# JasonHopeSpace/panda

Measured on AMD Instinct MI355X. Metric: MSM points/s (BN254, 2^24), higher is better.
Workload: dtype u32; 1 GPU; BN254 MSM 2^24 points per GPU, Jacobian output, bases and scalars resident in HBM; curve=bn254, log_points_per_gpu=24, exchange=none

## Files before the change

panda_amd/csrc/curve29.h:

```cpp
#pragma once
#include "fe29.h"

namespace panda29 {

template <class F>
struct Xyzz {
    Fe<F> X, Y, ZZ, ZZZ;
};

template <class F>
struct Bounds {
    static constexpr int M = SubMargin<F>::value;
    static constexpr int XB = 8 + M;
    static constexpr int YB = SubGrowth<F, 2>::value;
    static constexpr int PB = 2 + SubGrowth<F, XB>::value;
    static constexpr int RB = 2 + SubGrowth<F, YB>::value;
    static constexpr int VB = 2 + SubGrowth<F, XB>::value;
    static constexpr long long LIM = F::HEADROOM * 9 / 10;
    static_assert((long long)PB * PB < LIM, "P^2 exceeds the lazy-reduction headroom");
    static constexpr int NB = SubGrowth<F, 2>::value;
    static_assert((long long)RB * VB + (long long)YB * NB < LIM, "R*(Q-X3) - Y1*PPP exceeds the lazy-reduction headroom");
    static_assert(6LL * VB + 2LL * NB < LIM, "3x^2*(S-X3) - W*Y exceeds the lazy-reduction headroom");
    static_assert((long long)(2 * YB) * (2 * YB) < LIM, "(2Y)^2 exceeds the lazy-reduction headroom");
    static_assert(2 + SubGrowth<F, 6>::value <= XB, "X3 bound");
// ... 110 lines not shown
    fe_mul(U2, bx, acc.ZZ);
    fe_sub<F, B::XB>(P, U2, acc.X);
    fe_mul(S2, by, acc.ZZZ);
    fe_sub<F, B::YB>(R, S2, acc.Y);
    fe_sqr(PP, P);
    if (fe_is_zero_2p(PP))
        return fe_is_zero_mod_p(R) ? 1 : 2;
    fe_mul(PPP, P, PP);
    fe_mul(Q, acc.X, PP);
    fe_mul(acc.ZZ, acc.ZZ, PP);
    fe_mul(acc.ZZZ, acc.ZZZ, PPP);
    xyzz_finish(X3, Y3, R, Q, PPP, acc.Y);
    acc.X = X3;
    acc.Y = Y3;
    return 0;
}

template <class F>
struct SignedBounds {
    static constexpr double H = (double)F::HEADROOM;
    static constexpr double XS = 4.4, XN = 3.2, YS = 2.0, ZS = 2.0;
    static constexpr double XM = XS > XN ? XS : XN;
    static constexpr double PS = XM + ZS / H + 1, RS = YS + ZS / H + 1;
    static constexpr double PPS = PS * PS / H + 1, P3S = PS * PPS / H + 1, QS = XM * PPS / H + 1;
    static constexpr double RRS = RS * RS / H + 1, VS = QS + XM;
    static_assert(PPS < 2, "PP must stay below 2p for fe_is_zero_2p");
    static_assert(2 * QS + P3S < XN && RRS + 2 * QS + P3S < XS, "X3 leaves the accumulator's bound");
    static_assert((RS * VS + YS * P3S) / H + 1 < YS, "Y3 leaves the accumulator's bound");
    static_assert(ZS * PPS / H + 1 < ZS && ZS * P3S / H + 1 < ZS, "ZZ, ZZZ leave the accumulator's bound");
    static constexpr int KX = 4, KY = 1, KZZZ = 1;
    static_assert(XN < KX - 0.5 && XS + KX <= Bounds<F>::XB, "stored X after the conversion");
    static_assert((RS * VS + YS * P3S) / H < KY - 0.5 && YS + KY <= Bounds<F>::YB, "stored Y after the conversion");
    static_assert(ZS * P3S / H < KZZZ - 0.5 && ZS + KZZZ <= 3, "stored ZZZ after the conversion");
};

template <class F>
PANDA_HD void signed_after_doubling(Xyzz<F> &acc)
{
    fe_reduce_small_2p(acc.X);
}

template <class F>
PANDA_HD int xyzz_madd_core_s(Xyzz<F> &acc, const Fe<F> &bx, const Fe<F> &by)
{
    typedef SignedBounds<F> B;
    (void)sizeof(B);
    Fe<F> U2, S2, P, R, PP, PPP, Q, X3, Y3, t, rr, v, nppp;
    fe_mul(U2, bx, acc.ZZ);
    fe_sub_s(P, U2, acc.X);
    fe_mul_s(S2, by, acc.ZZZ);
    fe_sub_s(R, S2, acc.Y);
    fe_sqr_s(PP, P);
    if (fe_is_zero_2p(PP))
        return fe_is_zero_mod_p_s(R) ? 1 : 2;
    fe_mul_s(PPP, P, PP);
    fe_mul_s(Q, acc.X, PP);
    fe_mul(acc.ZZ, acc.ZZ, PP);
    fe_mul_s(acc.ZZZ, acc.ZZZ, PPP);
    fe_sqr_s(rr, R);
#if defined(__HIP_DEVICE_COMPILE__)
#pragma unroll
    for (int i = 0; i < F::N; i++) asm volatile("" : "+v"(Q.l[i]), "+v"(PPP.l[i]) : "v"(rr.l[F::N - 1]));
#endif
    fe_add_nr(t, Q, Q);
    fe_add_nr(t, t, PPP);
    fe_sub_s_wide(X3, rr, t);
    fe_norm_s(X3, X3);
    fe_sub_s(v, Q, X3);
    fe_neg_s(nppp, PPP);
    fe_mul_add_s(Y3, R, v, acc.Y, nppp);
    acc.X = X3;
    acc.Y = Y3;
    return 0;
}

template <class F>
PANDA_HD void xyzz_madd(Xyzz<F> &acc, const Fe<F> &bx, const Fe<F> &by, bool base_identity)
{
    if (base_identity) return;
    if (xyzz_is_identity(acc)) {
        xyzz_from_affine(acc, bx, by);
        return;
    }
    const int rare = xyzz_madd_core(acc, bx, by);
    if (rare == 1)
        xyzz_dbl_affine(acc, bx, by);
    else if (rare == 2)
        xyzz_set_identity(acc);
}

template <class F>
struct OutlineRareDoubling {
    static constexpr bool value = IsExt2<F>::value && F::N > 18;
};
template <class F>
#if defined(__HIPCC__)
__host__ __device__
#endif
__attribute__((noinline)) void xyzz_dbl_noinline(Xyzz<F> &r, const Xyzz<F> &p)
{
    xyzz_dbl(r, p);
}

template <class F>
PANDA_HD void xyzz_add(Xyzz<F> &acc, const Xyzz<F> &q)
{
// ... 118 lines not shown
```

panda_amd/csrc/fe29.h:

```cpp
#pragma once
#include <stdint.h>

#include "fe29_params.h"

#if defined(__HIPCC__)
#define PANDA_HD __host__ __device__ inline __attribute__((always_inline))
#else
#define PANDA_HD inline __attribute__((always_inline))
#endif

#if defined(FE29_CHECK)
#include <assert.h>
#define FE29_SHADOW_DECL unsigned __int128 shadow = 0;
#define FE29_SHADOW_MAC(x, y) shadow += (unsigned __int128)(x) * (y);
#define FE29_SHADOW_SHIFT()                                      \
    assert(shadow < ((unsigned __int128)1 << 64) && "fe29 column accumulator overflow"); \
    shadow >>= 29;
#else
#define FE29_SHADOW_DECL
#define FE29_SHADOW_MAC(x, y)
#define FE29_SHADOW_SHIFT()
#endif

#if defined(__HIP_DEVICE_COMPILE__) && !defined(FE29_NO_ASM)
// ... 204 lines not shown
template <class F, int K>
__device__ inline __attribute__((always_inline)) void fe29_mul_add_col_s(uint64_t &acc, const uint32_t *a, const uint32_t *b, const uint32_t *c, const uint32_t *d, uint32_t *m,
                                                                         uint32_t *out)
{
    constexpr int N = F::N;
    if constexpr (K == 0) {
        MacChain<1>::vvi0(acc, a, b);
        MacChain<1>::vvi(acc, c, d);
    } else if constexpr (K < N) {
        MacChain<K + 1>::vvi(acc, a, b + K);
        MacChain<K + 1>::vvi(acc, c, d + K);
    } else {
        MacChain<2 * N - 1 - K>::vvi(acc, a + (K - N + 1), b + (N - 1));
        MacChain<2 * N - 1 - K>::vvi(acc, c + (K - N + 1), d + (N - 1));
    }
    fe29_reduce_col<F, K, true>(acc, m, out);
}
template <class F, int... K>
__device__ inline __attribute__((always_inline)) void fe29_mul_cols_s(uint64_t &acc, const uint32_t *a, const uint32_t *b, uint32_t *m, uint32_t *out, std::integer_sequence<int, K...>)
{
    (fe29_mul_col_s<F, K>(acc, a, b, m, out), ...);
}
template <class F, int... K>
__device__ inline __attribute__((always_inline)) void fe29_sqr_cols_s(uint64_t &acc, const uint32_t *a, const uint32_t *a2, uint32_t *m, uint32_t *out, std::integer_sequence<int, K...>)
{
    (fe29_sqr_col_s<F, K>(acc, a, a2, m, out), ...);
}
template <class F, int... K>
__device__ inline __attribute__((always_inline)) void fe29_mul_add_cols_s(uint64_t &acc, const uint32_t *a, const uint32_t *b, const uint32_t *c, const uint32_t *d,
                                                                          uint32_t *m, uint32_t *out, std::integer_sequence<int, K...>)
{
    (fe29_mul_add_col_s<F, K>(acc, a, b, c, d, m, out), ...);
}
#endif

template <class F>
PANDA_HD void fe_mul(Fe<F> &r, const Fe<F> &a, const Fe<F> &b)
{
    constexpr int N = F::N;
    u32 m[N];
    u32 out[N];
    u64 acc = 0;
#if defined(FE29_DEVICE_CHAINS)
    fe29_mul_cols<F>(acc, a.l, b.l, m, out, std::make_integer_sequence<int, 2 * N - 1>());
    out[N - 1] = (u32)acc;
#pragma unroll
    for (int i = 0; i < N; i++) r.l[i] = out[i];
    return;
#endif
    FE29_SHADOW_DECL
#pragma unroll
    for (int k = 0; k < N; k++) {
#pragma unroll
        for (int i = 0; i <= k; i++) {
            FE29_MAC(acc, a.l[i], b.l[k - i]);
            FE29_SHADOW_MAC(a.l[i], b.l[k - i])
        }
#pragma unroll
        for (int i = 0; i < k; i++) {
            FE29_MAC_CONST(acc, m[i], F::P[k - i]);
            FE29_SHADOW_MAC(m[i], F::P[k - i])
        }
        m[k] = ((u32)acc * F::INV) & LIMB_MASK;
        FE29_MAC_CONST(acc, m[k], F::P[0]);
        FE29_SHADOW_MAC(m[k], F::P[0])
        acc >>= LIMB_BITS;
// ... 267 lines not shown
template <class F, int KB>
struct SubGrowth {
    static constexpr int value = F::KEFF[KB + SubMargin<F>::value];
};

template <class F, int KB>
PANDA_HD void fe_neg(Fe<F> &r, const Fe<F> &a)
{
    if constexpr (IsExt2<F>::value) {
        fe_neg<typename F::Base, KB>(ext_c0(r), ext_c0(a));
        fe_neg<typename F::Base, KB>(ext_c1(r), ext_c1(a));
        return;
    } else {
    constexpr int K = KB + SubMargin<F>::value;
    Fe<F> t;
#pragma unroll
    for (int i = 0; i < F::N; i++) {
#if defined(FE29_CHECK)
        assert(F::KP[K][i] >= a.l[i] && "fe_neg limb range");
#endif
        t.l[i] = F::KP[K][i] - a.l[i];
    }
    fe_norm(r, t);
    }
}

template <class F>
struct SignedLimbsOk {
    static constexpr bool value = !IsExt2<F>::value && F::N <= 9;
};
template <class F>
PANDA_HD constexpr bool fe_signed_columns_fit()
{
    return 2ull * F::N * ((u64)SLIMB_MAX * SLIMB_MAX) + (u64)F::N * (1ull << 58) + (1ull << 35) < (1ull << 63);
}

template <class F>
PANDA_HD void fe_mul_s(Fe<F> &r, const Fe<F> &a, const Fe<F> &b)
{
    constexpr int N = F::N;
    static_assert(SignedLimbsOk<F>::value && fe_signed_columns_fit<F>(), "signed column accumulator too narrow");
    u32 m[N];
    u32 out[N];
    u64 acc = 0;
#if defined(FE29_DEVICE_CHAINS)
    fe29_mul_cols_s<F>(acc, a.l, b.l, m, out, std::make_integer_sequence<int, 2 * N - 1>());
    out[N - 1] = (u32)acc;
#pragma unroll
    for (int i = 0; i < N; i++) r.l[i] = out[i];
    return;
#endif
    FE29_SHADOW_DECL_S
#pragma unroll
    for (int i = 0; i < N; i++) {
        FE29_CHECK_SLIMB(a.l[i]);
        FE29_CHECK_SLIMB(b.l[i]);
    }
#pragma unroll
    for (int k = 0; k < N; k++) {
#pragma unroll
        for (int i = 0; i <= k; i++) {
            FE29_MAC_S(acc, a.l[i], b.l[k - i]);
            FE29_SHADOW_MAC_S(a.l[i], b.l[k - i])
        }
#pragma unroll
        for (int i = 0; i < k; i++) {
            FE29_MAC_CONST(acc, m[i], F::P[k - i]);
// ... 129 lines not shown
        }
        m[k] = ((u32)acc * F::INV) & LIMB_MASK;
        FE29_MAC_CONST(acc, m[k], F::P[0]);
        FE29_SHADOW_MAC_S(m[k], F::P[0])
        FE29_SHADOW_SHIFT_S()
        acc = (u64)((int64_t)acc >> LIMB_BITS);
    }
#pragma unroll
    for (int k = N; k < 2 * N - 1; k++) {
#pragma unroll
        for (int i = k - N + 1; 2 * i < k; i++) {
            FE29_MAC_S(acc, a2[i], a.l[k - i]);
            FE29_SHADOW_MAC_S(a2[i], a.l[k - i])
        }
        if ((k & 1) == 0) {
            FE29_MAC_S(acc, a.l[k / 2], a.l[k / 2]);
            FE29_SHADOW_MAC_S(a.l[k / 2], a.l[k / 2])
        }
#pragma unroll
        for (int i = k - N + 1; i < N; i++) {
            FE29_MAC_CONST(acc, m[i], F::P[k - i]);
            FE29_SHADOW_MAC_S(m[i], F::P[k - i])
        }
        out[k - N] = (u32)acc & LIMB_MASK;
        FE29_SHADOW_SHIFT_S()
        acc = (u64)((int64_t)acc >> LIMB_BITS);
    }
    out[N - 1] = (u32)acc;
#pragma unroll
    for (int i = 0; i < N; i++) r.l[i] = out[i];
}

template <class F>
PANDA_HD void fe_sub_s(Fe<F> &r, const Fe<F> &a, const Fe<F> &b)
{
    static_assert(SignedLimbsOk<F>::value, "signed limbs: 9-limb prime fields only");
#pragma unroll
    for (int i = 0; i < F::N; i++) {
        r.l[i] = a.l[i] - b.l[i];
        FE29_CHECK_SLIMB(r.l[i]);
    }
}

template <class F>
PANDA_HD void fe_sub_s_wide(Fe<F> &r, const Fe<F> &a, const Fe<F> &b)
{
    static_assert(SignedLimbsOk<F>::value, "signed limbs: 9-limb prime fields only");
#pragma unroll
    for (int i = 0; i < F::N; i++) r.l[i] = a.l[i] - b.l[i];
}

template <class F>
PANDA_HD void fe_neg_s(Fe<F> &r, const Fe<F> &a)
{
    static_assert(SignedLimbsOk<F>::value, "signed limbs: 9-limb prime fields only");
#pragma unroll
    for (int i = 0; i < F::N; i++) r.l[i] = 0u - a.l[i];
}

template <class F>
PANDA_HD void fe_norm_s(Fe<F> &r, const Fe<F> &t)
{
    constexpr int N = F::N;
    static_assert(SignedLimbsOk<F>::value, "signed limbs: 9-limb prime fields only");
    u32 c[N];
#pragma unroll
    for (int i = 0; i < N - 1; i++) {
        c[i] = (u32)((int32_t)t.l[i] >> LIMB_BITS);
#if defined(FE29_CHECK)
        assert((int32_t)c[i] >= -3 && (int32_t)c[i] <= 1 && "fe_norm_s carry range");
#endif
    }
    u32 o[N];
    o[0] = t.l[0] & LIMB_MASK;
#pragma unroll
    for (int i = 1; i < N - 1; i++) o[i] = (t.l[i] & LIMB_MASK) + c[i - 1];
    o[N - 1] = t.l[N - 1] + c[N - 2];
#pragma unroll
    for (int i = 0; i < N; i++) r.l[i] = o[i];
}

template <class F>
PANDA_HD bool fe_is_zero_mod_p_s(const Fe<F> &a)
{
    static_assert(F::HEADROOM >= 160, "the bound above is BN254-like: R / p >= 160");
    Fe<F> one, t;
    fe_one(one);
    fe_mul_s(t, a, one);
    return fe_is_zero_2p(t);
}

template <class F, int K>
PANDA_HD void fe_from_signed(Fe<F> &r, const Fe<F> &a)
{
    static_assert(SignedLimbsOk<F>::value && K >= 1 && K <= 200, "signed limbs: 9-limb prime fields only");
    Fe<F> t;
#pragma unroll
    for (int i = 0; i < F::N; i++) {
#if defined(FE29_CHECK)
        assert((int64_t)(int32_t)a.l[i] + (int64_t)F::KP[K][i] >= 0 && (int64_t)(int32_t)a.l[i] + (int64_t)F::KP[K][i] < (1ll << 32) && "fe_from_signed limb range");
#endif
        t.l[i] = a.l[i] + F::KP[K][i];
    }
    fe_norm(r, t);
}

template <class F>
PANDA_HD void fe_unpack(Fe<F> &r, const u32 *w)
{
    constexpr int N = F::N, L = F::L;
#pragma unroll
    for (int k = 0; k < N; k++) {
        const int bit = 29 * k, wi = bit >> 5, sh = bit & 31;
        u32 v = 0;
        if (wi < L) {
            v = w[wi] >> sh;
            if (sh > 3 && wi + 1 < L) v |= w[wi + 1] << (32 - sh);
        }
        r.l[k] = (k < N - 1) ? (v & LIMB_MASK) : v;
    }
}

template <class F>
PANDA_HD void fe_pack(u32 *w, const Fe<F> &a)
{
    constexpr int N = F::N, L = F::L;
#pragma unroll
    for (int i = 0; i < L; i++) {
        const int bit = 32 * i, j = bit / 29, s = bit - 29 * j;
        u32 v = a.l[j] >> s;
        if (j + 1 < N) v |= a.l[j + 1] << (29 - s);
        if (29 - s + 29 < 32 && j + 2 < N) v |= a.l[j + 2] << (58 - s);
        w[i] = v;
    }
}
// ... 400 lines not shown
```

panda_amd/csrc/fe29_chain.h:

```cpp
#pragma once
#include <stdint.h>

namespace panda29 {

template <int CNT>
struct MacChain;

template <>
struct MacChain<1> {
    static __device__ inline __attribute__((always_inline)) void vv(uint64_t &acc, const uint32_t *x, const uint32_t *y)
    {
        asm("v_mad_u64_u32 %0, vcc, %1, %2, %0" : "+v"(acc) : "v"(x[0]), "v"(y[0]) : "vcc");
    }
    static __device__ inline __attribute__((always_inline)) void vs(uint64_t &acc, const uint32_t *x, const uint32_t *y)
    {
        asm("v_mad_u64_u32 %0, vcc, %1, %2, %0" : "+v"(acc) : "v"(x[0]), "s"(y[0]) : "vcc");
    }
    static __device__ inline __attribute__((always_inline)) void vv0(uint64_t &acc, const uint32_t *x, const uint32_t *y)
    {
        asm("v_mad_u64_u32 %0, vcc, %1, %2, 0" : "=&v"(acc) : "v"(x[0]), "v"(y[0]) : "vcc");
    }
    static __device__ inline __attribute__((always_inline)) void vs0(uint64_t &acc, const uint32_t *x, const uint32_t *y)
    {
        asm("v_mad_u64_u32 %0, vcc, %1, %2, 0" : "=&v"(acc) : "v"(x[0]), "s"(y[0]) : "vcc");
// ... 338 lines not shown
        asm("v_mad_u64_u32 %0, vcc, %1, %2, %0\n\tv_mad_u64_u32 %0, vcc, %3, %4, %0\n\tv_mad_u64_u32 %0, vcc, %5, %6, %0\n\tv_mad_u64_u32 %0, vcc, %7, %8, %0\n\tv_mad_u64_u32 %0, vcc, %9, %10, %0\n\tv_mad_u64_u32 %0, vcc, %11, %12, %0\n\tv_mad_u64_u32 %0, vcc, %13, %14, %0\n\tv_mad_u64_u32 %0, vcc, %15, %16, %0\n\tv_mad_u64_u32 %0, vcc, %17, %18, %0\n\tv_mad_u64_u32 %0, vcc, %19, %20, %0\n\tv_mad_u64_u32 %0, vcc, %21, %22, %0\n\tv_mad_u64_u32 %0, vcc, %23, %24, %0\n\tv_mad_u64_u32 %0, vcc, %25, %26, %0\n\tv_mad_u64_u32 %0, vcc, %27, %28, %0" : "+v"(acc) : "v"(x[0]), "v"(y[0]), "v"(x[1]), "v"(y[-1]), "v"(x[2]), "v"(y[-2]), "v"(x[3]), "v"(y[-3]), "v"(x[4]), "v"(y[-4]), "v"(x[5]), "v"(y[-5]), "v"(x[6]), "v"(y[-6]), "v"(x[7]), "v"(y[-7]), "v"(x[8]), "v"(y[-8]), "v"(x[9]), "v"(y[-9]), "v"(x[10]), "v"(y[-10]), "v"(x[11]), "v"(y[-11]), "v"(x[12]), "v"(y[-12]), "v"(x[13]), "v"(y[-13]) : "vcc");
    }
    static __device__ inline __attribute__((always_inline)) void vs(uint64_t &acc, const uint32_t *x, const uint32_t *y)
    {
        asm("v_mad_u64_u32 %0, vcc, %1, %2, %0\n\tv_mad_u64_u32 %0, vcc, %3, %4, %0\n\tv_mad_u64_u32 %0, vcc, %5, %6, %0\n\tv_mad_u64_u32 %0, vcc, %7, %8, %0\n\tv_mad_u64_u32 %0, vcc, %9, %10, %0\n\tv_mad_u64_u32 %0, vcc, %11, %12, %0\n\tv_mad_u64_u32 %0, vcc, %13, %14, %0\n\tv_mad_u64_u32 %0, vcc, %15, %16, %0\n\tv_mad_u64_u32 %0, vcc, %17, %18, %0\n\tv_mad_u64_u32 %0, vcc, %19, %20, %0\n\tv_mad_u64_u32 %0, vcc, %21, %22, %0\n\tv_mad_u64_u32 %0, vcc, %23, %24, %0\n\tv_mad_u64_u32 %0, vcc, %25, %26, %0\n\tv_mad_u64_u32 %0, vcc, %27, %28, %0" : "+v"(acc) : "v"(x[0]), "s"(y[0]), "v"(x[1]), "s"(y[-1]), "v"(x[2]), "s"(y[-2]), "v"(x[3]), "s"(y[-3]), "v"(x[4]), "s"(y[-4]), "v"(x[5]), "s"(y[-5]), "v"(x[6]), "s"(y[-6]), "v"(x[7]), "s"(y[-7]), "v"(x[8]), "s"(y[-8]), "v"(x[9]), "s"(y[-9]), "v"(x[10]), "s"(y[-10]), "v"(x[11]), "s"(y[-11]), "v"(x[12]), "s"(y[-12]), "v"(x[13]), "s"(y[-13]) : "vcc");
    }
    static __device__ inline __attribute__((always_inline)) void vv0(uint64_t &acc, const uint32_t *x, const uint32_t *y)
    {
        asm("v_mad_u64_u32 %0, vcc, %1, %2, 0\n\tv_mad_u64_u32 %0, vcc, %3, %4, %0\n\tv_mad_u64_u32 %0, vcc, %5, %6, %0\n\tv_mad_u64_u32 %0, vcc, %7, %8, %0\n\tv_mad_u64_u32 %0, vcc, %9, %10, %0\n\tv_mad_u64_u32 %0, vcc, %11, %12, %0\n\tv_mad_u64_u32 %0, vcc, %13, %14, %0\n\tv_mad_u64_u32 %0, vcc, %15, %16, %0\n\tv_mad_u64_u32 %0, vcc, %17, %18, %0\n\tv_mad_u64_u32 %0, vcc, %19, %20, %0\n\tv_mad_u64_u32 %0, vcc, %21, %22, %0\n\tv_mad_u64_u32 %0, vcc, %23, %24, %0\n\tv_mad_u64_u32 %0, vcc, %25, %26, %0\n\tv_mad_u64_u32 %0, vcc, %27, %28, %0" : "=&v"(acc) : "v"(x[0]), "v"(y[0]), "v"(x[1]), "v"(y[-1]), "v"(x[2]), "v"(y[-2]), "v"(x[3]), "v"(y[-3]), "v"(x[4]), "v"(y[-4]), "v"(x[5]), "v"(y[-5]), "v"(x[6]), "v"(y[-6]), "v"(x[7]), "v"(y[-7]), "v"(x[8]), "v"(y[-8]), "v"(x[9]), "v"(y[-9]), "v"(x[10]), "v"(y[-10]), "v"(x[11]), "v"(y[-11]), "v"(x[12]), "v"(y[-12]), "v"(x[13]), "v"(y[-13]) : "vcc");
    }
    static __device__ inline __attribute__((always_inline)) void vs0(uint64_t &acc, const uint32_t *x, const uint32_t *y)
    {
        asm("v_mad_u64_u32 %0, vcc, %1, %2, 0\n\tv_mad_u64_u32 %0, vcc, %3, %4, %0\n\tv_mad_u64_u32 %0, vcc, %5, %6, %0\n\tv_mad_u64_u32 %0, vcc, %7, %8, %0\n\tv_mad_u64_u32 %0, vcc, %9, %10, %0\n\tv_mad_u64_u32 %0, vcc, %11, %12, %0\n\tv_mad_u64_u32 %0, vcc, %13, %14, %0\n\tv_mad_u64_u32 %0, vcc, %15, %16, %0\n\tv_mad_u64_u32 %0, vcc, %17, %18, %0\n\tv_mad_u64_u32 %0, vcc, %19, %20, %0\n\tv_mad_u64_u32 %0, vcc, %21, %22, %0\n\tv_mad_u64_u32 %0, vcc, %23, %24, %0\n\tv_mad_u64_u32 %0, vcc, %25, %26, %0\n\tv_mad_u64_u32 %0, vcc, %27, %28, %0" : "=&v"(acc) : "v"(x[0]), "s"(y[0]), "v"(x[1]), "s"(y[-1]), "v"(x[2]), "s"(y[-2]), "v"(x[3]), "s"(y[-3]), "v"(x[4]), "s"(y[-4]), "v"(x[5]), "s"(y[-5]), "v"(x[6]), "s"(y[-6]), "v"(x[7]), "s"(y[-7]), "v"(x[8]), "s"(y[-8]), "v"(x[9]), "s"(y[-9]), "v"(x[10]), "s"(y[-10]), "v"(x[11]), "s"(y[-11]), "v"(x[12]), "s"(y[-12]), "v"(x[13]), "s"(y[-13]) : "vcc");
    }
    static __device__ inline __attribute__((always_inline)) void vvi(uint64_t &acc, const uint32_t *x, const uint32_t *y)
    {
        asm("v_mad_i64_i32 %0, vcc, %1, %2, %0\n\tv_mad_i64_i32 %0, vcc, %3, %4, %0\n\tv_mad_i64_i32 %0, vcc, %5, %6, %0\n\tv_mad_i64_i32 %0, vcc, %7, %8, %0\n\tv_mad_i64_i32 %0, vcc, %9, %10, %0\n\tv_mad_i64_i32 %0, vcc, %11, %12, %0\n\tv_mad_i64_i32 %0, vcc, %13, %14, %0\n\tv_mad_i64_i32 %0, vcc, %15, %16, %0\n\tv_mad_i64_i32 %0, vcc, %17, %18, %0\n\tv_mad_i64_i32 %0, vcc, %19, %20, %0\n\tv_mad_i64_i32 %0, vcc, %21, %22, %0\n\tv_mad_i64_i32 %0, vcc, %23, %24, %0\n\tv_mad_i64_i32 %0, vcc, %25, %26, %0\n\tv_mad_i64_i32 %0, vcc, %27, %28, %0" : "+v"(acc) : "v"(x[0]), "v"(y[0]), "v"(x[1]), "v"(y[-1]), "v"(x[2]), "v"(y[-2]), "v"(x[3]), "v"(y[-3]), "v"(x[4]), "v"(y[-4]), "v"(x[5]), "v"(y[-5]), "v"(x[6]), "v"(y[-6]), "v"(x[7]), "v"(y[-7]), "v"(x[8]), "v"(y[-8]), "v"(x[9]), "v"(y[-9]), "v"(x[10]), "v"(y[-10]), "v"(x[11]), "v"(y[-11]), "v"(x[12]), "v"(y[-12]), "v"(x[13]), "v"(y[-13]) : "vcc");
    }
    static __device__ inline __attribute__((always_inline)) void vvi0(uint64_t &acc, const uint32_t *x, const uint32_t *y)
    {
        asm("v_mad_i64_i32 %0, vcc, %1, %2, 0\n\tv_mad_i64_i32 %0, vcc, %3, %4, %0\n\tv_mad_i64_i32 %0, vcc, %5, %6, %0\n\tv_mad_i64_i32 %0, vcc, %7, %8, %0\n\tv_mad_i64_i32 %0, vcc, %9, %10, %0\n\tv_mad_i64_i32 %0, vcc, %11, %12, %0\n\tv_mad_i64_i32 %0, vcc, %13, %14, %0\n\tv_mad_i64_i32 %0, vcc, %15, %16, %0\n\tv_mad_i64_i32 %0, vcc, %17, %18, %0\n\tv_mad_i64_i32 %0, vcc, %19, %20, %0\n\tv_mad_i64_i32 %0, vcc, %21, %22, %0\n\tv_mad_i64_i32 %0, vcc, %23, %24, %0\n\tv_mad_i64_i32 %0, vcc, %25, %26, %0\n\tv_mad_i64_i32 %0, vcc, %27, %28, %0" : "=&v"(acc) : "v"(x[0]), "v"(y[0]), "v"(x[1]), "v"(y[-1]), "v"(x[2]), "v"(y[-2]), "v"(x[3]), "v"(y[-3]), "v"(x[4]), "v"(y[-4]), "v"(x[5]), "v"(y[-5]), "v"(x[6]), "v"(y[-6]), "v"(x[7]), "v"(y[-7]), "v"(x[8]), "v"(y[-8]), "v"(x[9]), "v"(y[-9]), "v"(x[10]), "v"(y[-10]), "v"(x[11]), "v"(y[-11]), "v"(x[12]), "v"(y[-12]), "v"(x[13]), "v"(y[-13]) : "vcc");
    }
};
template <>
struct MacChain<0> {
    static __device__ inline __attribute__((always_inline)) void vv(uint64_t &, const uint32_t *, const uint32_t *) {}
    static __device__ inline __attribute__((always_inline)) void vs(uint64_t &, const uint32_t *, const uint32_t *) {}
    static __device__ inline __attribute__((always_inline)) void vv0(uint64_t &acc, const uint32_t *, const uint32_t *) { acc = 0; }
    static __device__ inline __attribute__((always_inline)) void vvi(uint64_t &, const uint32_t *, const uint32_t *) {}
    static __device__ inline __attribute__((always_inline)) void vvi0(uint64_t &acc, const uint32_t *, const uint32_t *) { acc = 0; }
    static __device__ inline __attribute__((always_inline)) void vs0(uint64_t &acc, const uint32_t *, const uint32_t *) { acc = 0; }
};

}
```

panda_amd/csrc/msm_impl.h:

```cpp
#pragma once
#include <algorithm>
#include <vector>

#include "curve29_quad.h"
#include "msm_sort.h"
#include "panda_internal.h"

namespace panda {

struct MsmRegistration {
    const void *wire;
    void *converted;
    unsigned log_n, curve;
    int device;
    bool tabled;
    WindowPlan plan;
    size_t bytes;
    const uint32_t *samples;
    uint64_t hash;
};
hipError_t msm_hash_wire(const void *d_buf, size_t bytes, hipStream_t s, uint64_t *hash);

struct MsmTuning {
    unsigned window_bits;
// ... 273 lines not shown
        else hi = mid;
    }
    return lo;
}

__global__ void __launch_bounds__(256) k_chunk_first(const u32 *__restrict__ off, u32 *__restrict__ first, unsigned NB, unsigned K, unsigned chunks)
{
    const unsigned w = blockIdx.y;
    const u32 *ow = off + (u64)w * (NB + 1);
    u32 *fw = first + (u64)w * chunks;
    const unsigned b = blockIdx.x * blockDim.x + threadIdx.x;
    u32 t0 = 0, t1 = 0;
    if (b < NB) {
        const u32 lo = ow[b], hi = ow[b + 1];
        t0 = (lo + K - 1) / K;
        t1 = min((u32)((hi + K - 1) / K), (u32)chunks);
    }
    const unsigned lane = threadIdx.x & 63u;
    u64 wide = __ballot(t1 > t0 + 4);
    while (wide) {
        const int src = __ffsll((long long)wide) - 1;
        wide &= wide - 1;
        const u32 a = (u32)__shfl((int)t0, src), e = (u32)__shfl((int)t1, src), owner = (u32)__shfl((int)b, src);
        for (u32 t = a + lane; t < e; t += 64) fw[t] = owner;
    }
    if (t1 <= t0 + 4)
        for (u32 t = t0; t < t1; t++) fw[t] = b;
}

#ifndef PANDA_ROW_MASK
#define PANDA_ROW_MASK 0x7fffffffu
#endif
#ifndef PANDA_ACC_ITEMS
#define PANDA_ACC_ITEMS 0x7fu
#endif
constexpr unsigned ACC_ITEM_ROW_TUPLES = 32u;
constexpr unsigned ACC_ITEM_WORDS_NEG = 1u;
constexpr unsigned ACC_ITEM_Y_IDENTITY = 2u;
constexpr unsigned ACC_ITEM_QUAD_SHIFT = 4u;
constexpr unsigned ACC_ITEM_ID_FLAG = 8u;
constexpr unsigned ACC_ITEM_BOUNDARY = 16u;
constexpr unsigned ACC_ITEM_SIGNED_DIFF = 64u;
template <class F>
struct AccSlim {
    static constexpr bool value = !IsExt2<F>::value && F::N <= 9;
};
template <class F>
__host__ __device__ constexpr bool acc_item(unsigned item)
{
    return AccSlim<F>::value && (PANDA_ACC_ITEMS & item) != 0;
}
constexpr u32 STORED_SIGNED_MARK = 0x80000000u;
template <class F>
__device__ __forceinline__ void load_xyzz_stored(Xyzz<F> &p, const u32 *src)
{
    load_xyzz<F>(p, src);
    if constexpr (acc_item<F>(ACC_ITEM_SIGNED_DIFF)) {
        if (p.ZZ.l[F::N - 1] & STORED_SIGNED_MARK) {
            typedef SignedBounds<F> SB;
            p.ZZ.l[F::N - 1] &= ~STORED_SIGNED_MARK;
            fe_from_signed<F, SB::KX>(p.X, p.X);
            fe_from_signed<F, SB::KY>(p.Y, p.Y);
            fe_from_signed<F, SB::KZZZ>(p.ZZZ, p.ZZZ);
        }
    }
}

template <class F>
struct PackedBase {
    u32 w[2 * F::L];
};

template <class F>
__device__ __forceinline__ void fetch_base(PackedBase<F> &b, const u32 *bases, u32 entry)
{
#if defined(PANDA_ROWS_NT)
    load_words_stream<2 * F::L>(b.w, bases + (u64)(entry & PANDA_ROW_MASK) * 2 * F::L);
#else
    load_words<2 * F::L>(b.w, bases + (u64)(entry & PANDA_ROW_MASK) * 2 * F::L);
#endif
}

template <class F>
struct PackedRow {
    typedef u32 v4u __attribute__((ext_vector_type(4)));
    v4u q[2 * F::L / 4];
};
template <class F>
__device__ __forceinline__ void fetch_row(PackedRow<F> &r, const u32 *bases, u32 entry)
{
    typedef typename PackedRow<F>::v4u v4u;
    const v4u *s4 = reinterpret_cast<const v4u *>(bases + (u64)(entry & PANDA_ROW_MASK) * 2 * F::L);
#pragma unroll
    for (int j = 0; j < 2 * F::L / 4; j++) {
#if defined(PANDA_ROWS_NT)
        r.q[j] = __builtin_nontemporal_load(&s4[j]);
#else
        r.q[j] = s4[j];
#endif
    }
}
template <class F>
__device__ __forceinline__ void row_words(PackedBase<F> &b, const PackedRow<F> &r)
{
#pragma unroll
    for (int j = 0; j < 2 * F::L / 4; j++) {
        b.w[4 * j] = r.q[j].x;
        b.w[4 * j + 1] = r.q[j].y;
        b.w[4 * j + 2] = r.q[j].z;
        b.w[4 * j + 3] = r.q[j].w;
    }
}

template <class F, bool RAW = false, bool SLIM = false, bool LOCAL_P = false>
__device__ __forceinline__ void unpack_base(Fe<F> &x, Fe<F> &y, bool &inf, const PackedBase<F> &b, u32 entry)
{
    constexpr int L = F::L;
    constexpr bool WORDS_NEG = SLIM && acc_item<F>(ACC_ITEM_WORDS_NEG);
    constexpr int NZ_FROM = SLIM && acc_item<F>(ACC_ITEM_Y_IDENTITY) ? L : 0;
    u32 nz = 0;
#pragma unroll
    for (int k = NZ_FROM; k < 2 * L; k++) nz |= b.w[k];
    if constexpr (WORDS_NEG) asm volatile("" : "+v"(nz));
    inf = (nz == 0);
    fe_unpack(x, b.w);
    if constexpr (WORDS_NEG) {
        u32 yw[L];
#pragma unroll
        for (int k = 0; k < L; k++) yw[k] = b.w[L + k];
        if (entry >> 31) fe_words_neg<F, LOCAL_P>(yw, b.w + L);
        fe_unpack(y, yw);
    } else {
        fe_unpack(y, b.w + L);
        if (entry >> 31) {
            Fe<F> ny;
            if constexpr (RAW)
                fe_neg_raw<F, 1>(ny, y);
            else
                fe_neg<F, 1>(ny, y);
            y = ny;
        }
    }
}

#ifndef ACC_RAW_Y
#define ACC_RAW_Y false
#endif
struct AccPart {
    const u32 *pos;
    unsigned lo, hi, last, hi_bucket;
    u32 *queue;
};

template <class F>
__device__ __forceinline__ void fetch_base_lds(uint4 *lds_wave, const u32 *bases, u32 entry)
{
    const u32 *src = bases + (u64)(entry & PANDA_ROW_MASK) * 2 * F::L;
#pragma unroll
    for (int j = 0; j < 2 * F::L / 4; j++)
        __builtin_amdgcn_global_load_lds((const __attribute__((address_space(1))) void *)(src + 4 * j), (__attribute__((address_space(3))) void *)(lds_wave + j * 64), 16, 0, 0);
}
template <class F>
__device__ __forceinline__ void read_base_lds(PackedBase<F> &b, const uint4 *lds_wave, unsigned lane)
{
    asm volatile("s_waitcnt vmcnt(0)" ::: "memory");
#pragma unroll
    for (int j = 0; j < 2 * F::L / 4; j++) {
// ... 23 lines not shown
#pragma unroll
        for (int q = 0; q < 4; q++)
            __builtin_amdgcn_global_load_lds((const __attribute__((address_space(1))) void *)(src + 4 * q),
                                             (__attribute__((address_space(3))) void *)(lds_words + buffer * 256 + q * 64), 16, 0, 0);
    };
    uint4 quad = make_uint4(0, 0, 0, 0);
    if constexpr (SWLDS) {
        if (sectors) {
            sector_to_lds(0, sw + start);
            if (start + 16 < end) sector_to_lds(1, sw + start + 16);
            asm volatile("s_waitcnt vmcnt(0)" ::: "memory");
            quad = lds_words[lane];
        } else if (quads)
            quad = *reinterpret_cast<const uint4 *>(sw + start);
    } else if (quads)
        quad = *reinterpret_cast<const uint4 *>(sw + start);
    u32 cur_entry = quads ? quad.x : sw[start];
    u32 ahead_entry = quads ? quad.y : (start + 1 < end ? sw[start + 1] : 0u);
    constexpr bool ROW_TUPLES = !LDSROW && acc_item<F>(ACC_ITEM_ROW_TUPLES);
    constexpr int ROW_LOADS = 2 * F::L / 4;
    PackedRow<F> next_row;
    if constexpr (LDSROW)
        fetch_base_lds<F>(lds_wave, bases, cur_entry);
    else if constexpr (ROW_TUPLES)
        fetch_row<F>(next_row, bases, cur_entry);
    else
        fetch_base<F>(next_base, bases, cur_entry);
    constexpr bool QUAD_SHIFT = acc_item<F>(ACC_ITEM_QUAD_SHIFT);
    constexpr bool ID_FLAG = acc_item<F>(ACC_ITEM_ID_FLAG);
    constexpr bool SLIM_BOUNDARY = ID_FLAG && acc_item<F>(ACC_ITEM_BOUNDARY);
    constexpr bool Y_STORABLE = acc_item<F>(ACC_ITEM_WORDS_NEG) || !(ACC_RAW_Y && RawOperandOk<F>::value);
    constexpr bool SIGNED = acc_item<F>(ACC_ITEM_SIGNED_DIFF) && acc_item<F>(ACC_ITEM_WORDS_NEG) && !LDSROW;
    bool acc_id = true;
    u32 *brun = bw + (u64)b * PW;
    auto store_acc = [&](u32 *dst) {
        if constexpr (SIGNED) acc.ZZ.l[F::N - 1] |= (ID_FLAG ? acc_id : xyzz_is_identity(acc)) ? 0u : STORED_SIGNED_MARK;
        store_xyzz<F>(dst, acc);
    };
    if constexpr (QUAD_SHIFT) {
        quad.x = quad.y;
        quad.y = quad.z;
        quad.z = quad.w;
    }
    u32 trip = 0;
    for (u32 pos = start; pos < end; pos++, trip++) {
        Fe<F> cx, cy;
        bool cinf;
        const u32 entry = cur_entry;
        if constexpr (LDSROW) read_base_lds<F>(next_base, lds_wave, lane);
        if constexpr (ROW_TUPLES) row_words<F>(next_base, next_row);
        unpack_base<F, ACC_RAW_Y && RawOperandOk<F>::value, true, SIGNED>(cx, cy, cinf, next_base, entry);
        if constexpr (ROW_TUPLES) {
#pragma unroll
            for (int i = 0; i < F::N; i++) asm volatile("" : "+v"(cx.l[i]), "+v"(cy.l[i]));
        }
        const bool boundary = pos >= next;
        if (boundary) {
            if constexpr (SLIM_BOUNDARY) {
                store_acc(run_starts_inside ? brun : pw);
                run_starts_inside = true;
                do {
                    b++;
                    brun += PW;
                    next = ow[b + 1];
                } while (next <= pos);
                if (cinf) xyzz_set_identity(acc);
                acc_id = true;
            } else {
                store_acc(run_starts_inside ? bw + (u64)b * PW : pw);
                run_starts_inside = true;
                do {
                    b++;
                    next = ow[b + 1];
                } while (next <= pos);
                acc_id = cinf;
                if (cinf)
                    xyzz_set_identity(acc);
                else {
                    Fe<F> ty;
                    fe_norm(ty, cy);
                    xyzz_from_affine(acc, cx, ty);
                }
            }
        }
        if (pos + 1 < end) {
            cur_entry = ahead_entry;
            if constexpr (LDSROW)
                fetch_base_lds<F>(lds_wave, bases, cur_entry);
            else if constexpr (ROW_TUPLES)
                fetch_row<F>(next_row, bases, cur_entry);
            else
                fetch_base<F>(next_base, bases, cur_entry);
            if (pos + 2 < end) {
                if (quads) {
                    const u32 idx = QUAD_SHIFT ? trip + 2 : pos + 2 - start;
                    if ((idx & 3u) == 0) {
                        if (SWLDS && sectors) {
                            if ((idx & 15u) == 0) {
                                if (pos + 18 < end) {
                                    sector_to_lds((idx >> 4) + 1, sw + pos + 18);
                                    asm volatile("s_waitcnt vmcnt(%0)" ::"n"(ROW_LOADS + 4) : "memory");
                                } else
                                    asm volatile("s_waitcnt vmcnt(%0)" ::"n"(ROW_LOADS) : "memory");
                            }
                            quad = lds_words[((idx >> 4) & 1u) * 256 + ((idx >> 2) & 3u) * 64 + lane];
                        } else {
                            quad = *reinterpret_cast<const uint4 *>(sw + pos + 2);
                            if constexpr (ROW_TUPLES) asm volatile("" : "+v"(quad.x), "+v"(quad.y), "+v"(quad.z), "+v"(quad.w));
// ... 1 lines not shown
                    } else if constexpr (QUAD_SHIFT) {
                        quad.x = quad.y;
                        quad.y = quad.z;
                        quad.z = quad.w;
                    }
                    if constexpr (QUAD_SHIFT)
                        ahead_entry = quad.x;
                    else
                        ahead_entry = (idx & 2u) ? ((idx & 1u) ? quad.w : quad.z) : ((idx & 1u) ? quad.y : quad.x);
                } else {
                    ahead_entry = sw[pos + 2];
                    if constexpr (ROW_TUPLES) asm volatile("" : "+v"(ahead_entry));
                }
            }
        }
        if constexpr (!SLIM_BOUNDARY)
            if (boundary) continue;
        if (cinf) continue;
        if (ID_FLAG ? acc_id : xyzz_is_identity(acc)) {
            if constexpr (SLIM_BOUNDARY && Y_STORABLE) {
#pragma unroll
                for (int i = 0; i < F::N; i++) {
                    asm("v_mov_b32 %0, %1" : "=v"(acc.X.l[i]) : "v"(cx.l[i]));
                    asm("v_mov_b32 %0, %1" : "=v"(acc.Y.l[i]) : "v"(cy.l[i]));
                }
                fe_one(acc.ZZ);
                fe_one(acc.ZZZ);
            } else {
                Fe<F> ty;
                fe_norm(ty, cy);
                xyzz_from_affine(acc, cx, ty);
            }
            acc_id = false;
            continue;
        }
        int rare;
        if constexpr (SIGNED)
            rare = xyzz_madd_core_s(acc, cx, cy);
        else
            rare = xyzz_madd_core(acc, cx, cy);
        if (rare) {
            if (rare == 1) {
                PackedBase<F> again;
                const u32 same = acc_item<F>(ACC_ITEM_WORDS_NEG) ? sw[pos] : entry;
                fetch_base<F>(again, bases, same);
                unpack_base<F, false, true>(cx, cy, cinf, again, same);
                xyzz_dbl_affine(acc, cx, cy);
                if constexpr (SIGNED) signed_after_doubling(acc);
                acc_id = xyzz_is_identity(acc);
            } else {
                xyzz_set_identity(acc);
                acc_id = true;
            }
        }
    }
    const bool starts_inside = run_starts_inside;
    const bool ends_inside = next <= end;
    u32 *dst = (starts_inside && ends_inside) ? (SLIM_BOUNDARY ? brun : bw + (u64)b * PW) : (starts_inside ? pw + PW : pw);
    store_acc(dst);
}

template <class F, bool PERSIST, int WAVES = AccWaves<F>::value, bool LDSROW = false, bool SWLDS = false>
__global__ void __launch_bounds__(128, WAVES) k_accumulate(const u32 *__restrict__ bases, const u32 *__restrict__ sorted, const u32 *__restrict__ off,
                                                    u32 *__restrict__ bucket_acc, u32 *__restrict__ parts, u64 stride, unsigned NB, unsigned K,
                                                    unsigned chunks, u32 *__restrict__ long_count, const u32 *__restrict__ stale, AccPart part,
                                                    const u32 *__restrict__ chunk_first)
{
    constexpr int PW = 4 * F::N;
    const unsigned w = blockIdx.y;
    const unsigned t0 = blockIdx.x * blockDim.x + threadIdx.x;
    const u32 *fw = chunk_first ? chunk_first + (u64)w * chunks : nullptr;
    if (t0 == 0) long_count[w] = 0;
    if (stale && *stale) return;
    const u32 *ow = off + (u64)w * (NB + 1);
    const u32 lo_pos = part.pos ? part.pos[part.lo] : 0u;
    const u32 limit = part.pos ? part.pos[part.hi] : ow[NB];
    const unsigned search_hi = part.pos ? part.hi_bucket : NB;
    const bool takes_short_chunk = part.pos ? part.last != 0 : true;
    const u32 *sw = sorted + (u64)w * stride;
    u32 *bw = bucket_acc + (u64)w * NB * PW;
    __shared__ uint4 s_rows[LDSROW ? 2 * (2 * F::L / 4) * 64 : 1];
    uint4 *lds_wave = s_rows + (threadIdx.x >> 6) * (LDSROW ? (2 * F::L / 4) * 64 : 0);
    __shared__ uint4 s_words[SWLDS ? 2 * 512 : 1];
    uint4 *lds_words = s_words + (threadIdx.x >> 6) * (SWLDS ? 512 : 0);
    const unsigned lane = threadIdx.x & 63u;
    if constexpr (PERSIST) {
        const unsigned first = lo_pos / K;
// ... 978 lines not shown
```

Baseline: 1.023 billion points/s.

## Track accumulator sign lazily, fold X3 into squaring, add quick P==Q pre-check

Enables three new accumulate-kernel options by default. The first keeps a per-lane sign flag so the accumulator is stored possibly negated and the Y negation folds into the madd. The second fuses R^2 - 2Q - PPP into one signed squaring column chain. The third gates the full PP==0 test behind a wave ballot on the low limb. Together they remove separate negation, add and subtract passes from the hot mixed-add loop, at the cost of an extra conditional negate of the base Y, more flag bookkeeping, and changed bounds for stored values.

```diff
diff --git a/panda_amd/csrc/curve29.h b/panda_amd/csrc/curve29.h
--- a/panda_amd/csrc/curve29.h
+++ b/panda_amd/csrc/curve29.h
@@ -166,6 +166,9 @@
     static_assert(XN < KX - 0.5 && XS + KX <= Bounds<F>::XB, "stored X after the conversion");
     static_assert((RS * VS + YS * P3S) / H < KY - 0.5 && YS + KY <= Bounds<F>::YB, "stored Y after the conversion");
     static_assert(ZS * P3S / H < KZZZ - 0.5 && ZS + KZZZ <= 3, "stored ZZZ after the conversion");
+    static constexpr int KYN = 2;
+    static constexpr double YL = (RS * VS + YS * P3S) / H, YD = (6.0 * Bounds<F>::VB + Bounds<F>::NB) / H + 1;
+    static_assert(YL + 1 < KYN - 0.5 && YD < KYN - 0.5 && YL + KYN <= Bounds<F>::YB, "stored Y after the negating conversion");
 };
 
 template <class F>
@@ -174,7 +177,7 @@
     fe_reduce_small_2p(acc.X);
 }
 
-template <class F>
+template <class F, bool NEG_OUT = false, bool FOLD_X3 = false, bool QUICK_PQ = false>
 PANDA_HD int xyzz_madd_core_s(Xyzz<F> &acc, const Fe<F> &bx, const Fe<F> &by)
 {
     typedef SignedBounds<F> B;
@@ -185,27 +188,67 @@
     fe_mul_s(S2, by, acc.ZZZ);
     fe_sub_s(R, S2, acc.Y);
     fe_sqr_s(PP, P);
-    if (fe_is_zero_2p(PP))
-        return fe_is_zero_mod_p_s(R) ? 1 : 2;
+    if constexpr (QUICK_PQ) {
+#if defined(__HIP_DEVICE_COMPILE__)
+        if (__builtin_amdgcn_ballot_w64(PP.l[0] == 0 || PP.l[0] == F::P[0]) != 0)
+#else
+        if (PP.l[0] == 0 || PP.l[0] == F::P[0])
+#endif
+            if (fe_is_zero_2p(PP)) return fe_is_zero_mod_p_s(R) ? 1 : 2;
+    } else {
+        if (fe_is_zero_2p(PP)) return fe_is_zero_mod_p_s(R) ? 1 : 2;
+    }
     fe_mul_s(PPP, P, PP);
     fe_mul_s(Q, acc.X, PP);
     fe_mul(acc.ZZ, acc.ZZ, PP);
     fe_mul_s(acc.ZZZ, acc.ZZZ, PPP);
-    fe_sqr_s(rr, R);
+    if constexpr (FOLD_X3) {
+        fe_sqr_sub_s(X3, R, Q, PPP);
+    } else {
+        fe_sqr_s(rr, R);
 #if defined(__HIP_DEVICE_COMPILE__)
 #pragma unroll
-    for (int i = 0; i < F::N; i++) asm volatile("" : "+v"(Q.l[i]), "+v"(PPP.l[i]) : "v"(rr.l[F::N - 1]));
+        for (int i = 0; i < F::N; i++) asm volatile("" : "+v"(Q.l[i]), "+v"(PPP.l[i]) : "v"(rr.l[F::N - 1]));
 #endif
-    fe_add_nr(t, Q, Q);
-    fe_add_nr(t, t, PPP);
-    fe_sub_s_wide(X3, rr, t);
-    fe_norm_s(X3, X3);
-    fe_sub_s(v, Q, X3);
-    fe_neg_s(nppp, PPP);
-    fe_mul_add_s(Y3, R, v, acc.Y, nppp);
+        fe_add_nr(t, Q, Q);
+        fe_add_nr(t, t, PPP);
+        fe_sub_s_wide(X3, rr, t);
+        fe_norm_s(X3, X3);
+    }
+    if constexpr (NEG_OUT) {
+        fe_sub_s(v, X3, Q);
+        fe_mul_add_s(Y3, R, v, acc.Y, PPP);
+    } else {
+        fe_sub_s(v, Q, X3);
+        fe_neg_s(nppp, PPP);
+        fe_mul_add_s(Y3, R, v, acc.Y, nppp);
+    }
     acc.X = X3;
     acc.Y = Y3;
     return 0;
+}
+
+constexpr u32 STORED_SIGNED_MARK = 0x80000000u;
+constexpr u32 STORED_NEG_Y_MARK = 0x40000000u;
+template <class F>
+PANDA_HD void xyzz_mark_stored(Xyzz<F> &acc, bool identity, bool negated)
+{
+    acc.ZZ.l[F::N - 1] |= identity ? 0u : (negated ? STORED_SIGNED_MARK | STORED_NEG_Y_MARK : STORED_SIGNED_MARK);
+}
+template <class F>
+PANDA_HD void xyzz_from_stored(Xyzz<F> &p)
+{
+    typedef SignedBounds<F> SB;
+    const u32 top = p.ZZ.l[F::N - 1];
+    if (top & STORED_SIGNED_MARK) {
+        p.ZZ.l[F::N - 1] = top & ~(STORED_SIGNED_MARK | STORED_NEG_Y_MARK);
+        fe_from_signed<F, SB::KX>(p.X, p.X);
+        if (top & STORED_NEG_Y_MARK)
+            fe_from_signed<F, SB::KYN, true>(p.Y, p.Y);
+        else
+            fe_from_signed<F, SB::KY>(p.Y, p.Y);
+        fe_from_signed<F, SB::KZZZ>(p.ZZZ, p.ZZZ);
+    }
 }
 
 template <class F>
diff --git a/panda_amd/csrc/fe29.h b/panda_amd/csrc/fe29.h
--- a/panda_amd/csrc/fe29.h
+++ b/panda_amd/csrc/fe29.h
@@ -260,6 +260,27 @@
 {
     (fe29_mul_add_col_s<F, K>(acc, a, b, c, d, m, out), ...);
 }
+template <class F, int K>
+__device__ inline __attribute__((always_inline)) void fe29_sqr_sub_col_s(uint64_t &acc, const uint32_t *a, const uint32_t *a2, const uint32_t *q, const uint32_t *t, uint32_t *m,
+                                                                         uint32_t *out)
+{
+    constexpr int N = F::N;
+    constexpr int I0 = K < N ? 0 : K - N + 1;
+    constexpr int CNT = (K + 1) / 2 - I0;
+    MacChain<CNT>::vvi(acc, a2 + I0, a + (K - I0));
+    if constexpr (K == 0)
+        MacChain<1>::vvi0(acc, a, a);
+    else if constexpr ((K & 1) == 0)
+        MacChain<1>::vvi(acc, a + K / 2, a + K / 2);
+    if constexpr (K >= N) MacFold::sub_2x_y(acc, q + (K - N), t + (K - N));
+    fe29_reduce_col<F, K, true>(acc, m, out);
+}
+template <class F, int... K>
+__device__ inline __attribute__((always_inline)) void fe29_sqr_sub_cols_s(uint64_t &acc, const uint32_t *a, const uint32_t *a2, const uint32_t *q, const uint32_t *t, uint32_t *m,
+                                                                          uint32_t *out, std::integer_sequence<int, K...>)
+{
+    (fe29_sqr_sub_col_s<F, K>(acc, a, a2, q, t, m, out), ...);
+}
 #endif
 
 template <class F>
@@ -593,7 +614,7 @@
 template <class F>
 PANDA_HD constexpr bool fe_signed_columns_fit()
 {
-    return 2ull * F::N * ((u64)SLIMB_MAX * SLIMB_MAX) + (u64)F::N * (1ull << 58) + (1ull << 35) < (1ull << 63);
+    return 2ull * F::N * ((u64)SLIMB_MAX * SLIMB_MAX) + (u64)F::N * (1ull << 58) + (1ull << 35) + 3ull * SLIMB_MAX < (1ull << 63);
 }
 
 template <class F>
@@ -789,6 +810,87 @@
 }
 
 template <class F>
+PANDA_HD void fe_sqr_sub_s(Fe<F> &r, const Fe<F> &a, const Fe<F> &q, const Fe<F> &t)
+{
+    constexpr int N = F::N;
+    static_assert(SignedLimbsOk<F>::value && fe_signed_columns_fit<F>(), "signed column accumulator too narrow");
+    u32 m[N], out[N], a2[N];
+#pragma unroll
+    for (int i = 0; i < N; i++) a2[i] = a.l[i] << 1;
+    u64 acc = 0;
+#if defined(FE29_DEVICE_CHAINS)
+    fe29_sqr_sub_cols_s<F>(acc, a.l, a2, q.l, t.l, m, out, std::make_integer_sequence<int, 2 * N - 1>());
+    out[N - 1] = (u32)acc - (q.l[N - 1] << 1) - t.l[N - 1];
+#pragma unroll
+    for (int i = 0; i < N; i++) r.l[i] = out[i];
+    return;
+#endif
+    FE29_SHADOW_DECL_S
+#pragma unroll
+    for (int i = 0; i < N; i++) {
+        FE29_CHECK_SLIMB(a.l[i]);
+        FE29_CHECK_SLIMB(q.l[i]);
+        FE29_CHECK_SLIMB(t.l[i]);
+    }
+#pragma unroll
+    for (int k = 0; k < N; k++) {
+#pragma unroll
+        for (int i = 0; 2 * i < k; i++) {
+            FE29_MAC_S(acc, a2[i], a.l[k - i]);
+            FE29_SHADOW_MAC_S(a2[i], a.l[k - i])
+        }
+        if ((k & 1) == 0) {
+            FE29_MAC_S(acc, a.l[k / 2], a.l[k / 2]);
+            FE29_SHADOW_MAC_S(a.l[k / 2], a.l[k / 2])
+        }
+#pragma unroll
+        for (int i = 0; i < k; i++) {
+            FE29_MAC_CONST(acc, m[i], F::P[k - i]);
+            FE29_SHADOW_MAC_S(m[i], F::P[k - i])
+        }
+        m[k] = ((u32)acc * F::INV) & LIMB_MASK;
+        FE29_MAC_CONST(acc, m[k], F::P[0]);
+        FE29_SHADOW_MAC_S(m[k], F::P[0])
+        FE29_SHADOW_SHIFT_S()
+        acc = (u64)((int64_t)acc >> LIMB_BITS);
+    }
+#pragma unroll
+    for (int k = N; k < 2 * N - 1; k++) {
+#pragma unroll
+        for (int i = k - N + 1; 2 * i < k; i++) {
+            FE29_MAC_S(acc, a2[i], a.l[k - i]);
+            FE29_SHADOW_MAC_S(a2[i], a.l[k - i])
+        }
+        if ((k & 1) == 0) {
+            FE29_MAC_S(acc, a.l[k / 2], a.l[k / 2]);
+            FE29_SHADOW_MAC_S(a.l[k / 2], a.l[k / 2])
+        }
+#pragma unroll
+        for (int i = k - N + 1; i < N; i++) {
+            FE29_MAC_CONST(acc, m[i], F::P[k - i]);
+            FE29_SHADOW_MAC_S(m[i], F::P[k - i])
+        }
+        FE29_MAC_S(acc, q.l[k - N], -2);
+        FE29_SHADOW_MAC_S(q.l[k - N], -2)
+        FE29_MAC_S(acc, t.l[k - N], -1);
+        FE29_SHADOW_MAC_S(t.l[k - N], -1)
+        out[k - N] = (u32)acc & LIMB_MASK;
+        FE29_SHADOW_SHIFT_S()
+        acc = (u64)((int64_t)acc >> LIMB_BITS);
+    }
+    FE29_MAC_S(acc, q.l[N - 1], -2);
+    FE29_SHADOW_MAC_S(q.l[N - 1], -2)
+    FE29_MAC_S(acc, t.l[N - 1], -1);
+    FE29_SHADOW_MAC_S(t.l[N - 1], -1)
+#if defined(FE29_CHECK)
+    assert((int64_t)acc == (int64_t)shadow && (int64_t)acc == (int64_t)(int32_t)acc && "fe_sqr_sub_s top limb range");
+#endif
+    out[N - 1] = (u32)acc;
+#pragma unroll
+    for (int i = 0; i < N; i++) r.l[i] = out[i];
+}
+
+template <class F>
 PANDA_HD void fe_sub_s(Fe<F> &r, const Fe<F> &a, const Fe<F> &b)
 {
     static_assert(SignedLimbsOk<F>::value, "signed limbs: 9-limb prime fields only");
@@ -847,7 +949,7 @@
     return fe_is_zero_2p(t);
 }
 
-template <class F, int K>
+template <class F, int K, bool NEG = false>
 PANDA_HD void fe_from_signed(Fe<F> &r, const Fe<F> &a)
 {
     static_assert(SignedLimbsOk<F>::value && K >= 1 && K <= 200, "signed limbs: 9-limb prime fields only");
@@ -855,9 +957,10 @@
 #pragma unroll
     for (int i = 0; i < F::N; i++) {
 #if defined(FE29_CHECK)
-        assert((int64_t)(int32_t)a.l[i] + (int64_t)F::KP[K][i] >= 0 && (int64_t)(int32_t)a.l[i] + (int64_t)F::KP[K][i] < (1ll << 32) && "fe_from_signed limb range");
-#endif
-        t.l[i] = a.l[i] + F::KP[K][i];
+        const int64_t s = NEG ? -(int64_t)(int32_t)a.l[i] : (int64_t)(int32_t)a.l[i];
+        assert(s + (int64_t)F::KP[K][i] >= 0 && s + (int64_t)F::KP[K][i] < (1ll << 32) && "fe_from_signed limb range");
+#endif
+        t.l[i] = NEG ? F::KP[K][i] - a.l[i] : a.l[i] + F::KP[K][i];
     }
     fe_norm(r, t);
 }
diff --git a/panda_amd/csrc/fe29_chain.h b/panda_amd/csrc/fe29_chain.h
--- a/panda_amd/csrc/fe29_chain.h
+++ b/panda_amd/csrc/fe29_chain.h
@@ -394,4 +394,11 @@
     static __device__ inline __attribute__((always_inline)) void vs0(uint64_t &acc, const uint32_t *, const uint32_t *) { acc = 0; }
 };
 
+struct MacFold {
+    static __device__ inline __attribute__((always_inline)) void sub_2x_y(uint64_t &acc, const uint32_t *x, const uint32_t *y)
+    {
+        asm("v_mad_i64_i32 %0, vcc, %1, -2, %0\n\tv_mad_i64_i32 %0, vcc, %2, -1, %0" : "+v"(acc) : "v"(x[0]), "v"(y[0]) : "vcc");
+    }
+};
+
 }
diff --git a/panda_amd/csrc/msm_impl.h b/panda_amd/csrc/msm_impl.h
--- a/panda_amd/csrc/msm_impl.h
+++ b/panda_amd/csrc/msm_impl.h
@@ -329,7 +329,7 @@
 #define PANDA_ROW_MASK 0x7fffffffu
 #endif
 #ifndef PANDA_ACC_ITEMS
-#define PANDA_ACC_ITEMS 0x7fu
+#define PANDA_ACC_ITEMS 0x3ffu
 #endif
 constexpr unsigned ACC_ITEM_ROW_TUPLES = 32u;
 constexpr unsigned ACC_ITEM_WORDS_NEG = 1u;
@@ -338,6 +338,9 @@
 constexpr unsigned ACC_ITEM_ID_FLAG = 8u;
 constexpr unsigned ACC_ITEM_BOUNDARY = 16u;
 constexpr unsigned ACC_ITEM_SIGNED_DIFF = 64u;
+constexpr unsigned ACC_ITEM_SIGN_FLAG = 128u;
+constexpr unsigned ACC_ITEM_FOLD_X3 = 256u;
+constexpr unsigned ACC_ITEM_QUICK_PQ = 512u;
 template <class F>
 struct AccSlim {
     static constexpr bool value = !IsExt2<F>::value && F::N <= 9;
@@ -347,20 +350,11 @@
 {
     return AccSlim<F>::value && (PANDA_ACC_ITEMS & item) != 0;
 }
-constexpr u32 STORED_SIGNED_MARK = 0x80000000u;
 template <class F>
 __device__ __forceinline__ void load_xyzz_stored(Xyzz<F> &p, const u32 *src)
 {
     load_xyzz<F>(p, src);
-    if constexpr (acc_item<F>(ACC_ITEM_SIGNED_DIFF)) {
-        if (p.ZZ.l[F::N - 1] & STORED_SIGNED_MARK) {
-            typedef SignedBounds<F> SB;
-            p.ZZ.l[F::N - 1] &= ~STORED_SIGNED_MARK;
-            fe_from_signed<F, SB::KX>(p.X, p.X);
-            fe_from_signed<F, SB::KY>(p.Y, p.Y);
-            fe_from_signed<F, SB::KZZZ>(p.ZZZ, p.ZZZ);
-        }
-    }
+    if constexpr (acc_item<F>(ACC_ITEM_SIGNED_DIFF)) xyzz_from_stored(p);
 }
 
 template <class F>
@@ -409,11 +403,11 @@
     }
 }
 
-template <class F, bool RAW = false, bool SLIM = false, bool LOCAL_P = false>
+template <class F, bool RAW = false, bool SLIM = false, bool LOCAL_P = false, bool KEEP_Y = false>
 __device__ __forceinline__ void unpack_base(Fe<F> &x, Fe<F> &y, bool &inf, const PackedBase<F> &b, u32 entry)
 {
     constexpr int L = F::L;
-    constexpr bool WORDS_NEG = SLIM && acc_item<F>(ACC_ITEM_WORDS_NEG);
+    constexpr bool WORDS_NEG = SLIM && acc_item<F>(ACC_ITEM_WORDS_NEG) && !KEEP_Y;
     constexpr int NZ_FROM = SLIM && acc_item<F>(ACC_ITEM_Y_IDENTITY) ? L : 0;
     u32 nz = 0;
 #pragma unroll
@@ -429,7 +423,7 @@
         fe_unpack(y, yw);
     } else {
         fe_unpack(y, b.w + L);
-        if (entry >> 31) {
+        if (!KEEP_Y && (entry >> 31)) {
             Fe<F> ny;
             if constexpr (RAW)
                 fe_neg_raw<F, 1>(ny, y);
@@ -519,9 +513,13 @@
     constexpr bool Y_STORABLE = acc_item<F>(ACC_ITEM_WORDS_NEG) || !(ACC_RAW_Y && RawOperandOk<F>::value);
     constexpr bool SIGNED = acc_item<F>(ACC_ITEM_SIGNED_DIFF) && acc_item<F>(ACC_ITEM_WORDS_NEG) && !LDSROW;
     bool acc_id = true;
+    constexpr bool SIGN_FLAG = SIGNED && acc_item<F>(ACC_ITEM_SIGN_FLAG);
+    constexpr bool FOLD_X3 = SIGNED && acc_item<F>(ACC_ITEM_FOLD_X3);
+    constexpr bool QUICK_PQ = SIGNED && acc_item<F>(ACC_ITEM_QUICK_PQ);
+    bool acc_neg = false;
     u32 *brun = bw + (u64)b * PW;
     auto store_acc = [&](u32 *dst) {
-        if constexpr (SIGNED) acc.ZZ.l[F::N - 1] |= (ID_FLAG ? acc_id : xyzz_is_identity(acc)) ? 0u : STORED_SIGNED_MARK;
+        if constexpr (SIGNED) xyzz_mark_stored(acc, ID_FLAG ? acc_id : xyzz_is_identity(acc), SIGN_FLAG && acc_neg);
         store_xyzz<F>(dst, acc);
     };
     if constexpr (QUAD_SHIFT) {
@@ -536,7 +534,8 @@
         const u32 entry = cur_entry;
         if constexpr (LDSROW) read_base_lds<F>(next_base, lds_wave, lane);
         if constexpr (ROW_TUPLES) row_words<F>(next_base, next_row);
-        unpack_base<F, ACC_RAW_Y && RawOperandOk<F>::value, true, SIGNED>(cx, cy, cinf, next_base, entry);
+        unpack_base<F, ACC_RAW_Y && RawOperandOk<F>::value, true, SIGNED, SIGN_FLAG>(cx, cy, cinf, next_base, entry);
+        const bool neg = SIGN_FLAG && (entry >> 31) != 0;
         if constexpr (ROW_TUPLES) {
 #pragma unroll
             for (int i = 0; i < F::N; i++) asm volatile("" : "+v"(cx.l[i]), "+v"(cy.l[i]));
@@ -561,6 +560,7 @@
                     next = ow[b + 1];
                 } while (next <= pos);
                 acc_id = cinf;
+                acc_neg = neg;
                 if (cinf)
                     xyzz_set_identity(acc);
                 else {
@@ -628,27 +628,32 @@
                 xyzz_from_affine(acc, cx, ty);
             }
             acc_id = false;
+            acc_neg = neg;
             continue;
         }
         int rare;
-        if constexpr (SIGNED)
-            rare = xyzz_madd_core_s(acc, cx, cy);
-        else
+        if constexpr (SIGNED) {
+            if constexpr (SIGN_FLAG)
+                if (neg != acc_neg) fe_neg_s(cy, cy);
+            rare = xyzz_madd_core_s<F, SIGN_FLAG, FOLD_X3, QUICK_PQ>(acc, cx, cy);
+        } else
             rare = xyzz_madd_core(acc, cx, cy);
         if (rare) {
             if (rare == 1) {
                 PackedBase<F> again;
                 const u32 same = acc_item<F>(ACC_ITEM_WORDS_NEG) ? sw[pos] : entry;
                 fetch_base<F>(again, bases, same);
-                unpack_base<F, false, true>(cx, cy, cinf, again, same);
+                unpack_base<F, false, true, false, SIGN_FLAG>(cx, cy, cinf, again, same);
                 xyzz_dbl_affine(acc, cx, cy);
                 if constexpr (SIGNED) signed_after_doubling(acc);
                 acc_id = xyzz_is_identity(acc);
+                acc_neg = SIGN_FLAG && (same >> 31) != 0;
             } else {
                 xyzz_set_identity(acc);
                 acc_id = true;
             }
-        }
+        } else if constexpr (SIGN_FLAG)
+            acc_neg = !acc_neg;
     }
     const bool starts_inside = run_starts_inside;
     const bool ends_inside = next <= end;
```

Result: no change. 1.030 billion points/s (median of 6 runs) (+0.7%).
